# tansey/functionalmf

Measured on AMD Instinct MI355X. Metric: Gibbs sweeps/sec (full W+V update) at (512,256,64) K=5; % HBM roofline, higher is better.
Workload: dtype f64; 1 GPU; gaussian_btf c3 (512,256,64,4) nembeds=5 tf_order=2 complete data, W+V update, rng=device; burn_in_sweeps=10, step_loop=C side (btf_wv_steps: one call queues the K steps), v_sampler=spectral, likelihood_form=complete, parallelism=rows(W)/cols(V) x1

## Files before the change

### functionalmf_amd/csrc/btf_abi.hip

```cpp
#include "../../include/btf.h"
#include "btf_kernels.h"
#include "btf_banded_fast.h"
#include "btf_banded_twist.h"
#include "btf_banded_chunk.h"
#include "btf_spectral.h"
#include "btf_gass.h"
#include "btf_gass_ep.h"
#include "btf_gass_features.h"
#include "btf_gamma_grid.h"
#include "btf_fused.h"
#include "btf_functionals.h"
#include "btf_instances.h"
#include "btf_comm.h"
#include "btf_ctx.h"
#include <hip/hip_ext.h>
#include <unistd.h>

#include <algorithm>
#include <atomic>
#include <climits>
#include <cmath>
#include <cstdio>
#include <cstdlib>
#include <cstring>
// ... 142 lines not shown
  return BTF_OK;
}

inline int unr3_min_rpb() {
  static const int v = [] { const char* e = std::getenv("BTF_UNR3_RPB"); return e ? std::atoi(e) : 2048; }();
  return v;
}
inline bool lean_on() {
  static const bool v = [] { const char* e = std::getenv("BTF_ACC_LEAN"); return !e || std::atoi(e) != 0; }();
  return v;
}
template <int K>
void launch_accum(btf_ctx* c, int kid, int mode, const double* X, const double* Cx, const unsigned char* C8, const double* U,
                  const int* srcmap, int Rdim, int ld, int rpb, int nch, EigSide side = EigSide{nullptr, 0, 0, nullptr},
                  EigSideCols sidec = EigSideCols{nullptr, 0, CurveLists{nullptr, nullptr, nullptr}, nullptr, 0.0, nullptr},
                  TauSide tau = TauSide{}, GramSide gram = GramSide{},
                  ChunkMap cm = ChunkMap{0, 0, INT_MAX, 0, 0, 0}, SweepSide sw = SweepSide{},
                  const FuseW* fw = nullptr, const FuseV* fv = nullptr) {
  if (cm.row_end == 0) cm.row_end = Rdim;
  {
    static const double min_mb = [] { const char* e = std::getenv("BTF_NT_MIN_MB"); return e ? std::atof(e) : 100.0; }();
    cm.nt = (double)Rdim * (double)ld * 8.0 >= min_mb * 1048576.0 ? 1 : 0;
  }
#ifdef BTF_ACC_STAMPS
  cm.stamps = c->acc_stamps;
#endif
  Prof p(c, kid);
  const int cpw = TAU_SIDE_CPW;
  cm.nside = (sw.sc.hyp ? 1 : 0) + (sw.lam.hyp ? 1 : 0) + (side.out ? 1 + eig_side_groups(sidec.ncols, acc_waves(K, mode)) : 0) +
             (tau.Tau2 ? (tau.M + cpw - 1) / cpw : 0) + (gram.gpart ? gram.nblocks : 0) + (gram.sum_src ? 1 : 0) + (fw ? fw->owners : 0);
  dim3 grid((ld / ACC_TILE) * nch + cm.nside);
  if (fw || fv) {
    const bool unr3 = rpb >= unr3_min_rpb();
    if constexpr (K == 8) {
      if (unr3 && fw) { p.launch(accum_kernel<K, 0, 16, double, double, 3, 2, FUSE_W>, grid, dim3(16 * WAVE), 0, X, Cx, U, srcmap, c->part, Rdim, ld, rpb, side, sidec, tau, gram, cm, sw, *fw); return; }
      if (unr3 && fv) { p.launch(accum_kernel<K, 0, 16, double, double, 3, 2, FUSE_V>, grid, dim3(16 * WAVE), 0, X, Cx, U, srcmap, c->part, Rdim, ld, rpb, side, sidec, tau, gram, cm, sw, *fv); return; }
    }
    if constexpr (K <= 8) {
      if (fw) p.launch(accum_kernel<K, 0, 16, double, double, 0, 2, FUSE_W>, grid, dim3(16 * WAVE), 0, X, Cx, U, srcmap, c->part, Rdim, ld, rpb, side, sidec, tau, gram, cm, sw, *fw);
      else {
        const bool df_on = c->fused_dataflow != 0;
        FuseV f2 = *fv;
        constexpr int RG = K < 4 ? 4 : (K > 6 ? 6 : K);
        f2.dataflow = (df_on && f2.a.pband && f2.pimg && !f2.cnt && !f2.hp.flag && K <= 6 &&
                       vf_df_fits(f2.a.T, K, f2.a.TF, f2.a.nD, 16, RG)) ? 1 : 0;

        if constexpr (K <= 6) {
          if (f2.dataflow) { p.launch(accum_kernel<K, 0, 16, double, double, 0, 2, FUSE_VDF>, grid, dim3(16 * WAVE), 0, X, Cx, U, srcmap, c->part, Rdim, ld, rpb, side, sidec, tau, gram, cm, sw, f2); return; }
        }
        p.launch(accum_kernel<K, 0, 16, double, double, 0, 2, FUSE_V>, grid, dim3(16 * WAVE), 0, X, Cx, U, srcmap, c->part, Rdim, ld, rpb, side, sidec, tau, gram, cm, sw, f2);
      }
    }
    return;
  }
  const signed char* A8 = (mode >= 1 && !C8 && X == c->A_wT) ? c->A8_wT : ((mode >= 1 && !C8 && X == c->A_v) ? c->A8_v : nullptr);
  if (A8) {
    if (mode == 2) p.launch(accum_kernel<K, 2, acc_waves(K, 2), double, signed char>, grid, dim3(acc_waves(K, 2) * WAVE), 0, A8, Cx, U, srcmap, c->part, Rdim, ld, rpb, side, sidec, tau, gram, cm, sw, FuseNone{});
    else p.launch(accum_kernel<K, 1, acc_waves(K, 1), double, signed char>, grid, dim3(acc_waves(K, 1) * WAVE), 0, A8, Cx, U, srcmap, c->part, Rdim, ld, rpb, side, sidec, tau, gram, cm, sw, FuseNone{});
    return;
  }
  if (mode >= 1 && C8) {
    if (mode == 2) p.launch(accum_kernel<K, 2, acc_waves(K, 2), unsigned char>, grid, dim3(acc_waves(K, 2) * WAVE), 0, X, C8, U, srcmap, c->part, Rdim, ld, rpb, side, sidec, tau, gram, cm, sw, FuseNone{});
    else p.launch(accum_kernel<K, 1, acc_waves(K, 1), unsigned char>, grid, dim3(acc_waves(K, 1) * WAVE), 0, X, C8, U, srcmap, c->part, Rdim, ld, rpb, side, sidec, tau, gram, cm, sw, FuseNone{});
  } else if (mode == 2) p.launch(accum_kernel<K, 2>, grid, dim3(acc_waves(K, 2) * WAVE), 0, X, Cx, U, srcmap, c->part, Rdim, ld, rpb, side, sidec, tau, gram, cm, sw, FuseNone{});
  else if (mode == 1) p.launch(accum_kernel<K, 1>, grid, dim3(acc_waves(K, 1) * WAVE), 0, X, Cx, U, srcmap, c->part, Rdim, ld, rpb, side, sidec, tau, gram, cm, sw, FuseNone{});
  else if (K <= 8 && acc_waves(K, 0) == 16 && rpb < unr3_min_rpb() && !tau.Tau2 && !sw.sc.hyp && !sw.lam.hyp && lean_on()) {
    if constexpr (K <= 8) p.launch(accum_kernel<K, 0, 16, double, double, 0, 2, FUSE_LEAN>, grid, dim3(16 * WAVE), 0, X, Cx, U, srcmap, c->part, Rdim, ld, rpb, side, sidec, tau, gram, cm, sw, FuseNone{});
  }
  else if (K >= 10 && ACC_WAVES != acc_waves(10, 0) && !side.out && rpb < unr3_min_rpb()) {
    if constexpr (K >= 10) p.launch(accum_kernel<K, 0, ACC_WAVES>, grid, dim3(ACC_WAVES * WAVE), 0, X, Cx, U, srcmap, c->part, Rdim, ld, rpb, side, sidec, tau, gram, cm, sw, FuseNone{});
  }
  else if (rpb >= unr3_min_rpb()) p.launch(accum_kernel<K, 0, acc_waves(K, 0), double, double, 3>, grid, dim3(acc_waves(K, 0) * WAVE), 0, X, Cx, U, srcmap, c->part, Rdim, ld, rpb, side, sidec, tau, gram, cm, sw, FuseNone{});
  else p.launch(accum_kernel<K, 0>, grid, dim3(acc_waves(K, 0) * WAVE), 0, X, Cx, U, srcmap, c->part, Rdim, ld, rpb, side, sidec, tau, gram, cm, sw, FuseNone{});
}
struct PgPasses { bool flat, series, frac; int mode; };
PgPasses pg_passes(const btf_ctx* c) {
  PgPasses p{false, false, false, c->pg_mode};
  if (c->counts && p.mode == PG_MODE_DEFAULT) p.mode = PG_MODE_SERIES_ALL;
  if (p.mode == PG_MODE_SERIES_ALL) { p.series = true; return p; }
  if (p.mode == PG_MODE_EXACT_ALL) { p.flat = c->pg_has_small || c->pg_has_big; p.frac = c->pg_has_frac; }
  else { p.flat = c->pg_has_small; p.series = c->pg_has_big || c->pg_has_frac; }
  if (!p.flat && !p.series && !p.frac) p.series = true;
  return p;
}
template <int K>
void launch_pg(btf_ctx* c, const double* B, double* out, const double* Lf, const double* Uf, int nl, int ld, int Rdim,
               unsigned long long base, unsigned long long stride_r, unsigned long long stride_l, unsigned long long seed) {
  const int gx = (nl + PG_THREADS - 1) / PG_THREADS;
  int nrb = std::max(1, std::min(Rdim, 4096 / std::max(1, gx)));
  const int rpb = (Rdim + nrb - 1) / nrb;
  nrb = (Rdim + rpb - 1) / rpb;
  const PgPasses ps = pg_passes(c);
  int fill = 1;
  if (ps.flat) {
    Prof p(c, BTF_K_PG);
    const int rpx = round_up(rpb, PGX_CPL);
// ... 3766 lines not shown
```

### functionalmf_amd/csrc/btf_fused.h

```cpp
#pragma once
#include "btf_kernels.h"
#include "btf_spectral.h"

namespace btf {

__device__ __forceinline__ bool poll_flag(const unsigned* flag, unsigned epoch) {
  for (unsigned spins = 0; spins < (1u << 22); ++spins) {
    if (__hip_atomic_load((const gu32_t*)flag, __ATOMIC_RELAXED, __HIP_MEMORY_SCOPE_AGENT) == epoch) return true;
    __builtin_amdgcn_s_sleep(8);
  }
  return false;
}

struct HypPub { const double* pub; const unsigned* flag; unsigned epoch; int which; };

struct FuseW {
  WSolveArgs a;
  unsigned* cnt;
  unsigned expected;
  int owners;
  int rows;
  int rw;
  HypPub hp;
  const unsigned* gram_cnt; unsigned gram_expected;
// ... 771 lines not shown
template <> __device__ __forceinline__ unsigned* fuse_tickets<FUSE_VDF>(const FuseV& fz) { return nullptr; }
template <> __device__ __forceinline__ int fuse_chunks<FUSE_VDF>(const FuseV& fz) { return 1; }
template <> __device__ __forceinline__ int fuse_owners<FUSE_VDF>(const FuseV&) { return 0; }

__device__ __forceinline__ void df_signal(unsigned* c) {
  __builtin_amdgcn_fence(__ATOMIC_RELEASE, "workgroup");
  if ((threadIdx.x & 63) == 0) __hip_atomic_fetch_add(c, 1u, __ATOMIC_RELAXED, __HIP_MEMORY_SCOPE_WORKGROUP);
}
#ifndef BTF_DF_SLEEP
#define BTF_DF_SLEEP 1
#endif
template <int SLEEP = BTF_DF_SLEEP>
__device__ __forceinline__ void df_wait(unsigned* c, unsigned target, unsigned* bad) {
  bool seen = false;
  for (unsigned spins = 0; spins < (1u << 22) / SLEEP; ++spins) {
    if (__hip_atomic_load(c, __ATOMIC_RELAXED, __HIP_MEMORY_SCOPE_WORKGROUP) >= target) { seen = true; break; }
    __builtin_amdgcn_s_sleep(SLEEP);
  }
  if (!seen && (threadIdx.x & 63) == 0) __hip_atomic_store(bad, 1u, __ATOMIC_RELAXED, __HIP_MEMORY_SCOPE_WORKGROUP);
  __builtin_amdgcn_fence(__ATOMIC_ACQUIRE, "workgroup");
}

template <int K, int S>
__device__ __forceinline__ void v_df_begin(const FuseV& fv, int tile, double* lds, VDfPre& pre) {
  unsigned* cw = reinterpret_cast<unsigned*>(lds + vf_red_doubles(false) - VF_MAILBOX + 96);
  if (threadIdx.x < 64) cw[threadIdx.x] = 0u;
  __syncthreads();
  v_df_band_load<K, S>(fv, tile, pre);
}
template <int K, int S>
__device__ __forceinline__ void v_df_band_load(const FuseV& fv, int tile, VDfPre& pre) {
  const VSpecArgs& a = fv.a;
  const int T = a.T, NG = ACC_TILE / T;
  const int lane = threadIdx.x & 63;
  const int pw = __builtin_amdgcn_readfirstlane(threadIdx.x >> 6);
  const int cg = pw - NG, j = tile * NG + cg;
#pragma unroll
  for (int u = 0; u < 8; ++u) pre.pv[u] = make_double2(0.0, 0.0);
  if (pw >= NG && pw < 2 * NG && j < a.ml) {
    const int PB = df_layout(T, K, S).PB;
    const double2* src = reinterpret_cast<const double2*>(fv.pimg + (size_t)j * 2 * PB);
#pragma unroll
    for (int u = 0; u < 8; ++u)
      if (lane + 64 * u < PB) pre.pv[u] = src[lane + 64 * u];
  }
}
template <int K, int S>
__device__ __forceinline__ void v_df_band_store(const FuseV& fv, int tile, double* lds, const VDfPre& pre) {
  const VSpecArgs& a = fv.a;
  const int T = a.T, NG = ACC_TILE / T;
  const int lane = threadIdx.x & 63;
  const int pw = __builtin_amdgcn_readfirstlane(threadIdx.x >> 6);
  const int cg = pw - NG;
  if (!(pw >= NG && pw < 2 * NG && tile * NG + cg < a.ml)) return;
  const DfLayout D = df_layout(T, K, S);
  double2* dst = reinterpret_cast<double2*>(lds + vf_red_doubles(false) - VF_MAILBOX - (size_t)(cg + 1) * D.size + D.P);
#pragma unroll
  for (int u = 0; u < 8; ++u)
    if (lane + 64 * u < D.PB) dst[lane + 64 * u] = pre.pv[u];
  unsigned* cw = reinterpret_cast<unsigned*>(lds + vf_red_doubles(false) - VF_MAILBOX + 96);
  df_signal(cw + DFC_GROUP0 + cg * DFC_PER_GROUP + DFG_BAND);
}

template <int K, int S, int WAVES, int RG, int NVV>
__device__ __forceinline__ void v_fused_df(const FuseV& fv, int tile, double* lds, const double (&acc)[NVV][2], long long* stamps,
                                           const DfEarly& early) {
  static_assert(NVV == K && K <= RG, "one reduction round");
  static_assert(S == 3 && WAVES == 16, "tf_order 2, 16 waves");
  VSpecArgs a = fv.a;
  const int T = a.T, n = T * K, KK = tri(K);
  constexpr int D1 = S + 1, WN = S * (S + 1) + S;
  constexpr int NT = VF_GROUP_WAVES * WAVE;
  const int NG = ACC_TILE / T;
  const int Tp = T + S + 1;
  int nl, nr, ns;
  spectral_split(T, S, nl, nr, ns);
  const int lane = threadIdx.x & 63;
// ... 360 lines not shown
```

### functionalmf_amd/csrc/btf_instances.h

```cpp
#pragma once
#include "btf_kernels.h"
#include "btf_banded_twist.h"
#include "btf_spectral.h"
#include "btf_fused.h"

namespace btf {

#define BTF_ACC_ARGS_F(XT, CT, FZ) \
  (const XT*, const CT*, const double*, const int*, double*, int, int, int, EigSide, EigSideCols, TauSide, GramSide, ChunkMap, SweepSide, FZ)
#define BTF_ACC_ARGS(XT, CT) BTF_ACC_ARGS_F(XT, CT, FuseNone)
#define BTF_ACCUM_SET(P, K)                                                                              \
  P void accum_kernel<K, 0> BTF_ACC_ARGS(double, double);                                                \
  P void accum_kernel<K, 0, acc_waves(K, 0), double, double, 3> BTF_ACC_ARGS(double, double);            \
  P void accum_kernel<K, 1> BTF_ACC_ARGS(double, double);                                                \
  P void accum_kernel<K, 2> BTF_ACC_ARGS(double, double);                                                \
  P void accum_kernel<K, 1, acc_waves(K, 1), unsigned char> BTF_ACC_ARGS(double, unsigned char);         \
  P void accum_kernel<K, 2, acc_waves(K, 2), unsigned char> BTF_ACC_ARGS(double, unsigned char);         \
  P void accum_kernel<K, 1, acc_waves(K, 1), double, signed char> BTF_ACC_ARGS(signed char, double);     \
  P void accum_kernel<K, 2, acc_waves(K, 2), double, signed char> BTF_ACC_ARGS(signed char, double);

#define BTF_ACCUM_K10W_SET(P)                                                                            \
  P void accum_kernel<10, 0, ACC_WAVES> BTF_ACC_ARGS(double, double);

#define BTF_FUSED_W_SET(P, K)                                                                            \
  P void accum_kernel<K, 0, 16, double, double, 0, 2, FUSE_W> BTF_ACC_ARGS_F(double, double, FuseW);
#define BTF_FUSED_V_SET(P, K)                                                                            \
  P void accum_kernel<K, 0, 16, double, double, 0, 2, FUSE_V> BTF_ACC_ARGS_F(double, double, FuseV);
#define BTF_FUSED_VDF_SET(P, K)                                                                          \
  P void accum_kernel<K, 0, 16, double, double, 0, 2, FUSE_VDF> BTF_ACC_ARGS_F(double, double, FuseV);
#define BTF_LEAN_SET(P, K)                                                                               \
  P void accum_kernel<K, 0, 16, double, double, 0, 2, FUSE_LEAN> BTF_ACC_ARGS(double, double);
#define BTF_FUSED_UNR3_SET(P, K)                                                                         \
// ... 91 lines not shown
```

### functionalmf_amd/csrc/btf_kernels.h

```cpp
#pragma once
#include <type_traits>
#include "btf_device.h"
#include "btf_eig.h"
#include "btf_pg_exact.h"

namespace btf {

#ifndef BTF_ACC_WAVES
#define BTF_ACC_WAVES 16
#endif
#ifndef BTF_DF_UNR
#define BTF_DF_UNR 4
#endif
#ifndef BTF_DF_PREFETCH
#define BTF_DF_PREFETCH 1
#endif
#ifndef BTF_DF_SHARE
#define BTF_DF_SHARE 0
#endif
#ifndef BTF_ACC_UNR
#define BTF_ACC_UNR 2
#endif
#ifndef BTF_ACC_PF_WT
#define BTF_ACC_PF_WT 0
#endif
#ifndef BTF_ACC_UNR_WT
#define BTF_ACC_UNR_WT 2
#endif
#ifndef BTF_ACC_WAVES_WT
#define BTF_ACC_WAVES_WT 12
#endif
#ifndef BTF_ACC_WAVES_K10
#define BTF_ACC_WAVES_K10 8
#endif
#ifndef BTF_ACC_UNR_K9
#define BTF_ACC_UNR_K9 2
#endif
#ifndef BTF_ACC_ULDS_MINK
// ... 141 lines not shown

struct EigSideCols { const int* cols; int ncols; CurveLists cv; const double* W; double inv_R; double* eig_cols; };
__host__ __device__ constexpr int eig_side_tpw(int waves) { return waves >= 4 ? 4 : waves; }
__host__ __device__ constexpr int eig_side_groups(int ncols, int waves) { return (ncols + eig_side_tpw(waves) - 1) / eig_side_tpw(waves); }

struct TauSide {
  const double* V; int T, nD, M;
  const int* dr_ptr; const int* dr_col; const double* dr_val;
  double lam2, lo, hi;
  double* Tau2; double* Ta; double* Tb; double* Tc; double* lsum;
  unsigned long long seed; const double* hyp;
};
__device__ void tau2_column(const TauSide& t, int K, int j, int tid256, double* red4);
constexpr int TAU_SIDE_CPW = 2;

struct GramSide {
  const double* U; int Rdim; double* gpart; int nblocks; unsigned* cnt;
  const double* sum_src; int sum_n; double* sum_out; int sum_threads;
};

struct ChunkMap {
  int slot_base, row_base, skip_at, skip_rows, row_end; int nside;
  int nt;
#ifdef BTF_ACC_STAMPS
  long long* stamps;
#endif
};

struct ScalarSide {
  const double* sse_cols; int M; double sconst, nobs;
  const double* W; int NK; double nfree;
  double nu2_a, nu2_b, sig_a, sig_b; int which; unsigned long long seed; double* hyp;
  double* pub; unsigned* flag; unsigned epoch;
};
struct LamSide { const double* lsum; int M; double shape; int exact; unsigned long long seed; double* hyp; double* pub; unsigned* flag; unsigned epoch; };
struct SweepSide { ScalarSide sc; LamSide lam; };
struct BandSide {
  const double* Tau2; int nD;
  const int* st_ptr; const int* st_row; const double* st_coef;
  int TD1, col0, ml;
  double* pband; double* pimg; int img_T, img_D1, img_PB;
  const double* hyp; double lam2;
  const double* lam_pub; const unsigned* lam_flag; unsigned epoch;
  int* status;
};
__device__ inline void band_side(const BandSide& bs, int j, double* itau, int nthreads);
// ... 35 lines not shown
struct VPre;
template <int K, int S, int WAVES, int NSUM>
__device__ __forceinline__ void v_fused_tail(const FuseV& fv, int tile, double* lds, const double (&sums)[NSUM], int nv_round, int tv, int tc, long long* stamps,
                                             const VPre& pre, const double* mailbox, bool band_early, bool unr3);
template <int K, int S> __device__ __forceinline__ void v_fused_prefetch(const FuseV& fv, int tile, double* mailbox, VPre& pre, bool band_early);
template <int K, int S, class PRE> __device__ __forceinline__ void v_fused_prefetch_loads(const FuseV& fv, int tile, PRE& pre, bool band_early);
constexpr int VF_PRE = 4;
template <int K, int S> __device__ __forceinline__ bool v_fused_band_early(const FuseV& fv, int tile, double* lds, bool unr3);
#ifndef BTF_VF_BANDPRE
#define BTF_VF_BANDPRE 1
#endif
#if BTF_VF_BANDPRE
template <int K, int S> __device__ __forceinline__ bool v_fused_band_preload(const FuseV& fv, int tile, VPre& pre);
template <int K, int S> __device__ __forceinline__ void v_fused_band_store(const FuseV& fv, int tile, double* lds, const VPre& pre, bool unr3);
#endif
template <int FUSE> struct FusePre { struct type {}; };
constexpr int VF_MAILBOX_DOUBLES = 128;
struct VDfPre { double2 pv[8]; };
template <int FUSE> __device__ __forceinline__ int fuse_chain_waves(const typename FuseSel<FUSE>::type& fz) { return 0; }
struct DfEarly { double epub; bool have; };
template <int FUSE> __device__ __forceinline__ const unsigned* fuse_eig_flag(const typename FuseSel<FUSE>::type& fz) { return nullptr; }
template <int FUSE> __device__ __forceinline__ const double* fuse_eig_pub(const typename FuseSel<FUSE>::type& fz) { return nullptr; }
template <int FUSE> __device__ __forceinline__ unsigned fuse_epoch(const typename FuseSel<FUSE>::type& fz) { return 0u; }
template <int K, int S> __device__ __forceinline__ void v_df_begin(const FuseV& fv, int tile, double* lds, VDfPre& pre);
template <int K, int S> __device__ __forceinline__ void v_df_band_load(const FuseV& fv, int tile, VDfPre& pre);
template <int K, int S> __device__ __forceinline__ void v_df_band_store(const FuseV& fv, int tile, double* lds, const VDfPre& pre);
template <int K, int S, int WAVES, int RG, int NVV>
__device__ __forceinline__ void v_fused_df(const FuseV& fv, int tile, double* lds, const double (&acc)[NVV][2], long long* stamps, const DfEarly& early);
template <int FUSE> __device__ __forceinline__ unsigned* fuse_tickets(const typename FuseSel<FUSE>::type& fz);
template <int FUSE> __device__ __forceinline__ int fuse_chunks(const typename FuseSel<FUSE>::type& fz);
__device__ __forceinline__ bool last_arriver_of(unsigned* cnt, unsigned expected, unsigned* word) {
  if (threadIdx.x == 0) {
    const unsigned t = __hip_atomic_fetch_add((gu32_t*)cnt, 1u, __ATOMIC_RELAXED, __HIP_MEMORY_SCOPE_AGENT);
    const bool last = t + 1u == expected;
    if (last) __hip_atomic_store((gu32_t*)cnt, 0u, __ATOMIC_RELAXED, __HIP_MEMORY_SCOPE_AGENT);
    *word = last ? 1u : 0u;
  }
  __syncthreads();
  const bool last = *word != 0u;
  __syncthreads();
  return last;
}
__host__ __device__ constexpr int vf_red_doubles(bool unr3) { return unr3 ? 15360 : 18432; }
__host__ __device__ constexpr int w_tail_lds_doubles(int K);
__host__ __device__ constexpr int w_owner_lds_budget(int K);

#ifdef BTF_ACC_STAMPS
#define ACC_STAMP(i) do { if (threadIdx.x == 0 && b < 4096 && cm.stamps) cm.stamps[b * 8 + (i)] = wall_clock64(); } while (0)
#define ACC_SIDE_STAMP(i) do { if (threadIdx.x == 0 && cm.stamps) cm.stamps[(4096 + blockIdx.x) * 8 + (i)] = wall_clock64(); } while (0)
#define ACC_TAIL_STAMPS (cm.stamps && b < 4096 ? cm.stamps + b * 8 : nullptr)
#define ACC_OWNER_STAMPS (cm.stamps ? cm.stamps + (size_t)(4096 + blockIdx.x) * 8 : nullptr)
#else
#define ACC_STAMP(i) do { } while (0)
#define ACC_SIDE_STAMP(i) do { } while (0)
#define ACC_TAIL_STAMPS nullptr
#define ACC_OWNER_STAMPS nullptr
#endif
#define TAIL_STAMP(st, i) do { if ((st) && threadIdx.x == 0) (st)[i] = wall_clock64(); } while (0)
template <int K, int MODE, int WAVES = acc_waves(K, MODE), typename CT = double, typename XT = double, int UNRV = 0,
          int OPL = acc_opl(K, MODE), int FUSE = FUSE_NONE>
__global__ __launch_bounds__(WAVES * WAVE) BTF_ACC_EU_ATTR(K, MODE, WAVES, FUSE) void accum_kernel(
    const XT* __restrict__ X, const CT* __restrict__ Cx, const double* __restrict__ U,
    const int* __restrict__ srcmap, double* __restrict__ part, int Rdim, int ld,
    int rows_per_block, EigSide side, EigSideCols sidec, TauSide tau, GramSide gram, ChunkMap cm, SweepSide sw,
    typename FuseSel<FUSE>::type fz) {
  static_assert(FUSE == FUSE_NONE || (MODE == 0 && OPL == 2 && WAVES == 16), "the fused tails follow the complete-data stream");
  constexpr bool PLAIN = FUSE == FUSE_NONE || FUSE == FUSE_LEAN;
  constexpr int KK = tri(K);
  constexpr int NV = MODE == 0 ? K : K + KK;
  constexpr int ACC_WAVES = WAVES;
  constexpr int ACC_UNR = FUSE == FUSE_VDF ? BTF_DF_UNR : (UNRV > 0 ? UNRV : (MODE >= 1 ? BTF_ACC_UNR_WT : (K >= 9 ? BTF_ACC_UNR_K9 : BTF_ACC_UNR)));
  constexpr int ACC_RGT = WAVES * WAVE / ACC_TILE, ACC_RGL = (96 * 1024) / (WAVES * ACC_TILE * 8);
  constexpr int ACC_RG0 = ACC_RGT < 4 ? ACC_RGT : 4;
  constexpr int ACC_RGW = ACC_RGT < ACC_RGL ? (ACC_RGT < NV ? ACC_RGT : NV) : (ACC_RGL < NV ? ACC_RGL : NV);
  constexpr int ACC_RG = ACC_RGW > ACC_RG0 ? ACC_RGW : ACC_RG0;
  constexpr int RED_SLOT = ACC_RG * ACC_TILE;
  constexpr int RED_SLOTS = (FUSE == FUSE_V || FUSE == FUSE_VDF) ? (vf_red_doubles(UNRV == 3) + RED_SLOT - 1) / RED_SLOT : ACC_WAVES;
  static_assert(RED_SLOTS >= ACC_WAVES, "reduction scratch");
  __shared__ double red[RED_SLOTS][ACC_RG][ACC_TILE];
  static_assert(FUSE != FUSE_W || (w_tail_lds_doubles(K) <= WAVES * ACC_RG * ACC_TILE && w_owner_lds_budget(K) == WAVES * ACC_RG * ACC_TILE), "W owner scratch");
  constexpr bool ULDS = MODE == 0 && K >= BTF_ACC_ULDS_MINK && UNRV == 3;
  constexpr int ACC_UROWS_MAX = 512;
  __shared__ double ush[ULDS ? ACC_UROWS_MAX * K : 1];

  const int lane = threadIdx.x & 63;
  const int wave = __builtin_amdgcn_readfirstlane(threadIdx.x >> 6);
  int b = blockIdx.x;
  if (b < cm.nside) {
  if constexpr (FUSE == FUSE_W) {
    const int nown = fuse_owners<FUSE>(fz);
    if (b < nown) {
      ACC_SIDE_STAMP(0);
      w_fused_owner<K, WAVES>(fz, b, &red[0][0][0], ACC_OWNER_STAMPS);
      ACC_SIDE_STAMP(3);
      return;
    }
    b -= nown;
  }
  if constexpr (FUSE != FUSE_LEAN) {
  if (sw.sc.hyp) {
    if (b == 0) { sweep_scalar_side<WAVES>(sw.sc, &red[0][0][0]); return; }
    b -= 1;
  }
  if (sw.lam.hyp) {
    if (b == 0) { sweep_lam_side<WAVES>(sw.lam, &red[0][0][0]); return; }
    b -= 1;
  }
  }
  if (side.out) {
    constexpr int TPW = eig_side_tpw(WAVES);
    const int nside = 1 + eig_side_groups(sidec.ncols, WAVES);
// ... 76 lines not shown
      if ((int)threadIdx.x < gram.sum_threads && l < lanes) {
        double sg = 0.0;
        for (int b0 = l; b0 < gram.sum_n; b0 += 8 * lanes) {
          double x[8];
#pragma unroll
          for (int u = 0; u < 8; ++u) x[u] = b0 + u * lanes < gram.sum_n ? gram.sum_src[(size_t)(b0 + u * lanes) * KK + q] : 0.0;
#pragma unroll
          for (int u = 0; u < 8; ++u) sg += x[u];
        }
        scratch[l * KK + q] = sg;
      }
      __syncthreads();
      if ((int)threadIdx.x < KK) {
        double t = 0.0;
        for (int bb = 0; bb < lanes; ++bb) t += scratch[bb * KK + threadIdx.x];
        gram.sum_out[threadIdx.x] = t;
      }
      return;
    }
    b -= 1;
  }
  return;
  }
  b -= cm.nside;
  ACC_STAMP(0);
  const int ntiles = ld / ACC_TILE;
  const int lchunk = b / ntiles, tile = b - lchunk * ntiles;
  const int chunk = cm.slot_base + lchunk;
  static_assert(OPL == 2 || (OPL == 1 && WAVES % 2 == 0), "outputs per lane");
  constexpr int NWR = OPL == 2 ? WAVES : WAVES / 2;
  const int half = OPL == 2 ? 0 : (wave & 1);
  const int wv = OPL == 2 ? wave : (wave >> 1);
  const size_t col = (size_t)tile * ACC_TILE + (OPL == 2 ? 2 * lane : 64 * half + lane);
  int r0 = cm.row_base + lchunk * rows_per_block;
  if (r0 >= cm.skip_at) r0 += cm.skip_rows;
  const int r1 = min(r0 + rows_per_block, cm.row_end);

  constexpr bool dataflow = FUSE == FUSE_VDF;
  static_assert(!dataflow || (UNRV != 3 && NV <= ACC_RG && OPL == 2), "the dataflow tail: one reduction round, two rows in flight");
  bool df_band_done = false;
  DfEarly df_early{0.0, false};
  VDfPre dfpre;
  if constexpr (dataflow) v_df_begin<K, 3>(fz, tile, &red[0][0][0], dfpre);
  int df_ncw = 0;
  if constexpr (dataflow) df_ncw = fuse_chain_waves<FUSE>(fz);
  int nwr_rt = NWR;
  bool band_early = false;
  if constexpr (FUSE == FUSE_V) band_early = v_fused_band_early<K, 3>(fz, tile, &red[0][0][0], UNRV == 3);
  typename FusePre<FUSE>::type vpre;
#if BTF_VF_BANDPRE
  if constexpr (FUSE == FUSE_V) band_early = v_fused_band_preload<K, 3>(fz, tile, vpre);
#endif
  double acc[NV][OPL];
#pragma unroll
  for (int v = 0; v < NV; ++v)
#pragma unroll
    for (int o = 0; o < OPL; ++o) acc[v][o] = 0.0;
#ifdef BTF_NO_NT
  constexpr bool nt = false;
#else
  const bool nt = __builtin_amdgcn_readfirstlane(cm.nt) != 0;
#endif
  int s0 = 0, s1 = 0;
  bool gram_on = true, gram_any = true;
  if constexpr (MODE == 2) {
    s0 = srcmap[col];
    if constexpr (OPL == 2) s1 = srcmap[col + 1];
    const bool own = s0 == (int)col || (OPL == 2 && s1 == (int)col + 1);
    gram_on = __builtin_amdgcn_readfirstlane(__any(own) ? 1 : 0) != 0;
    if constexpr (OPL == 1) gram_any = __syncthreads_or(own ? 1 : 0) != 0;
    else gram_any = gram_on;
  }
  int cs_form = 0, cs_src = 0;
  if constexpr (MODE == 2 && OPL == 2) {
    cs_src = __builtin_amdgcn_readfirstlane(s0);
    if (__all(s0 == cs_src && s1 == cs_src)) cs_form = 1;
    else if (__all(s1 == s0 + 1 && (s0 & 1) == 0)) cs_form = 2;
    cs_form = __builtin_amdgcn_readfirstlane(cs_form);
  }

  int ublk0 = r0;
  struct Rows { double2 x[ACC_UNR]; double2 c[MODE >= 1 ? ACC_UNR : 1]; double2 cs[MODE == 2 ? ACC_UNR : 1]; double uk[ACC_UNR][K]; };
  auto load_rows = [&](int rb, Rows& R, auto full, auto ntc) {
    constexpr bool FULL = decltype(full)::value;
// ... 121 lines not shown
      if (!nextB) break;
      more = rb + STEP < full_end;
      if (more) load_rows(rb + STEP, A, std::true_type{}, ntc);
      compute(rb, B);
      rb += STEP;
    }
  } else {
    if constexpr (FUSE == FUSE_V) {
      const int pre_end = full_end - VF_PRE * STEP;
      for (; rb < pre_end; rb += STEP) {
        Rows A;
        load_rows(rb, A, std::true_type{}, ntc);
        compute(rb, A);
      }
      v_fused_prefetch_loads<K, 3>(fz, tile, vpre, band_early);
    }
    if constexpr (dataflow) {
      const int g1 = NWR * ACC_UNR;
      const int rsplit = r0 + ((r1 - r0) * BTF_DF_SHARE / 100) / g1 * g1;
      nwr_rt = NWR;
      for (rb = r0 + wv; rb < rsplit; rb += g1) {
        Rows A;
        load_rows(rb, A, std::true_type{}, ntc);
        compute(rb, A);
        if (!df_band_done) { v_df_band_store<K, 3>(fz, tile, &red[0][0][0], dfpre); df_band_done = true; }
      }
      if (wave >= df_ncw) {
        nwr_rt = NWR - df_ncw;
        const int step = nwr_rt * ACC_UNR, fend = r1 - (ACC_UNR - 1) * nwr_rt;
        const bool eigw = BTF_DF_PREFETCH && wave == df_ncw;
        const int rprobe = r0 + (r1 - r0) * 5 / 8;
        unsigned eflag = 0u;
        int estate = 0;
        for (rb = rsplit + wv - df_ncw; rb < fend; rb += step) {
          Rows A;
          load_rows(rb, A, std::true_type{}, ntc);
          if (eigw && estate < 2 && rb >= rprobe) {
            if (estate == 1 && eflag == fuse_epoch<FUSE>(fz)) {
              if (lane < K + K * K) df_early.epub = load_sc1(fuse_eig_pub<FUSE>(fz) + lane);
              df_early.have = true;
              estate = 2;
            } else {
              eflag = __hip_atomic_load(fuse_eig_flag<FUSE>(fz), __ATOMIC_RELAXED, __HIP_MEMORY_SCOPE_AGENT);
              estate = 1;
            }
          }
          compute(rb, A);
          if (!df_band_done) { v_df_band_store<K, 3>(fz, tile, &red[0][0][0], dfpre); df_band_done = true; }
        }
        if (rb < r1) {
          Rows A;
          load_rows(rb, A, std::false_type{}, ntc);
          compute(rb, A);
        }
      }
      rb = r1;
    }
    for (; rb < full_end; rb += STEP) {
      Rows A;
      load_rows(rb, A, std::true_type{}, ntc);
      compute(rb, A);
    }
  }
  if constexpr (!ULDS) {
    if (rb < r1) {
      Rows A;
      load_rows(rb, A, std::false_type{}, ntc);
      compute(rb, A);
    }
  }

  };
  if (nt) run_stream(std::true_type{}); else run_stream(std::false_type{});
  ACC_STAMP(2);
  if constexpr (dataflow) {
    if (!df_band_done) {
      v_df_band_load<K, 3>(fz, tile, dfpre);
      v_df_band_store<K, 3>(fz, tile, &red[0][0][0], dfpre);
    }
    v_fused_df<K, 3, WAVES, ACC_RG, NV>(fz, tile, &red[0][0][0], acc, ACC_TAIL_STAMPS, df_early);
    return;
  }
  if constexpr (FUSE == FUSE_V) {
    if constexpr (ULDS) v_fused_prefetch_loads<K, 3>(fz, tile, vpre, band_early);
#if BTF_VF_BANDPRE
    if (band_early) v_fused_band_store<K, 3>(fz, tile, &red[0][0][0], vpre, UNRV == 3);
#endif
    v_fused_prefetch<K, 3>(fz, tile, &red[0][0][0] + RED_SLOTS * RED_SLOT - VF_MAILBOX_DOUBLES, vpre, band_early);
  }
  const int tv = threadIdx.x >> 7;
  const int tc = threadIdx.x & 127;
  constexpr int NFS = PLAIN ? 1 : (NV + ACC_RG - 1) / ACC_RG;
  double fsum[NFS];
#pragma unroll
  for (int r = 0; r < NFS; ++r) fsum[r] = 0.0;
#pragma unroll
  for (int g = 0; g < NV; g += ACC_RG) {
    if (MODE == 2 && !gram_any && g >= K) break;
#pragma unroll
    for (int v = 0; v < ACC_RG; ++v) {
      if (g + v < NV) {
// ... 2341 lines not shown
```

Baseline: 26790 sweeps/s.

## Repack accum kernel arguments into a compact preloaded head and defer dataflow LDS init

Reorders and compresses the accumulate kernel's argument list so the hot scalars (pointers, ld, rows, row_end, packed nside/flags/T code) fit in a fixed 14-dword head. The intent is that the kernel reads them from preloaded SGPRs instead of loading ChunkMap and FuseV fields from the kernarg segment. Row remapping is now skipped behind a flag, and the dataflow band load takes pimg, T and ml directly. The mailbox-zeroing barrier in v_df_begin is moved until after the first row loads are issued, so it no longer stalls the stream start. The risks are the ABI change across every instance and a changed placement of __syncthreads relative to the loads.

Result: no change. 26980 sweeps/s, median of 2 (+0.7%).

```diff
diff --git a/functionalmf_amd/csrc/btf_abi.hip b/functionalmf_amd/csrc/btf_abi.hip
--- a/functionalmf_amd/csrc/btf_abi.hip
+++ b/functionalmf_amd/csrc/btf_abi.hip
@@ -188,22 +188,26 @@
     static const double min_mb = [] { const char* e = std::getenv("BTF_NT_MIN_MB"); return e ? std::atof(e) : 100.0; }();
     cm.nt = (double)Rdim * (double)ld * 8.0 >= min_mb * 1048576.0 ? 1 : 0;
   }
+  AccRest rest{cm.slot_base, cm.row_base, cm.skip_at, cm.skip_rows};
+  const bool remap = cm.slot_base != 0 || cm.row_base != 0 || cm.skip_rows != 0;
+  const unsigned long long aux2 = (unsigned long long)reinterpret_cast<uintptr_t>(srcmap);
 #ifdef BTF_ACC_STAMPS
-  cm.stamps = c->acc_stamps;
+  rest.stamps = c->acc_stamps;
 #endif
   Prof p(c, kid);
   const int cpw = TAU_SIDE_CPW;
   cm.nside = (sw.sc.hyp ? 1 : 0) + (sw.lam.hyp ? 1 : 0) + (side.out ? 1 + eig_side_groups(sidec.ncols, acc_waves(K, mode)) : 0) +
              (tau.Tau2 ? (tau.M + cpw - 1) / cpw : 0) + (gram.gpart ? gram.nblocks : 0) + (gram.sum_src ? 1 : 0) + (fw ? fw->owners : 0);
   dim3 grid((ld / ACC_TILE) * nch + cm.nside);
+  const unsigned nside_flags = ((unsigned)cm.nside << ACC_F_BITS) | (cm.nt ? ACC_F_NT : 0u) | (remap ? ACC_F_REMAP : 0u);
   if (fw || fv) {
     const bool unr3 = rpb >= unr3_min_rpb();
     if constexpr (K == 8) {
-      if (unr3 && fw) { p.launch(accum_kernel<K, 0, 16, double, double, 3, 2, FUSE_W>, grid, dim3(16 * WAVE), 0, X, Cx, U, srcmap, c->part, Rdim, ld, rpb, side, sidec, tau, gram, cm, sw, *fw); return; }
-      if (unr3 && fv) { p.launch(accum_kernel<K, 0, 16, double, double, 3, 2, FUSE_V>, grid, dim3(16 * WAVE), 0, X, Cx, U, srcmap, c->part, Rdim, ld, rpb, side, sidec, tau, gram, cm, sw, *fv); return; }
+      if (unr3 && fw) { p.launch(accum_kernel<K, 0, 16, double, double, 3, 2, FUSE_W>, grid, dim3(16 * WAVE), 0, X, U, c->part, (const void*)Cx, aux2, ld, rpb, cm.row_end, nside_flags, rest, side, sidec, tau, gram, sw, *fw); return; }
+      if (unr3 && fv) { p.launch(accum_kernel<K, 0, 16, double, double, 3, 2, FUSE_V>, grid, dim3(16 * WAVE), 0, X, U, c->part, (const void*)Cx, aux2, ld, rpb, cm.row_end, nside_flags, rest, side, sidec, tau, gram, sw, *fv); return; }
     }
     if constexpr (K <= 8) {
-      if (fw) p.launch(accum_kernel<K, 0, 16, double, double, 0, 2, FUSE_W>, grid, dim3(16 * WAVE), 0, X, Cx, U, srcmap, c->part, Rdim, ld, rpb, side, sidec, tau, gram, cm, sw, *fw);
+      if (fw) p.launch(accum_kernel<K, 0, 16, double, double, 0, 2, FUSE_W>, grid, dim3(16 * WAVE), 0, X, U, c->part, (const void*)Cx, aux2, ld, rpb, cm.row_end, nside_flags, rest, side, sidec, tau, gram, sw, *fw);
       else {
         const bool df_on = c->fused_dataflow != 0;
         FuseV f2 = *fv;
@@ -212,32 +216,33 @@
                        vf_df_fits(f2.a.T, K, f2.a.TF, f2.a.nD, 16, RG)) ? 1 : 0;
 
         if constexpr (K <= 6) {
-          if (f2.dataflow) { p.launch(accum_kernel<K, 0, 16, double, double, 0, 2, FUSE_VDF>, grid, dim3(16 * WAVE), 0, X, Cx, U, srcmap, c->part, Rdim, ld, rpb, side, sidec, tau, gram, cm, sw, f2); return; }
+          if (f2.dataflow) { p.launch(accum_kernel<K, 0, 16, double, double, 0, 2, FUSE_VDF>, grid, dim3(16 * WAVE), 0, X, U, c->part, (const void*)f2.pimg, (unsigned long long)f2.a.ml, ld, rpb, cm.row_end,
+                                      nside_flags | (acc_depth_code(f2.a.T) << ACC_F_T_SHIFT), rest, side, sidec, tau, gram, sw, f2); return; }
         }
-        p.launch(accum_kernel<K, 0, 16, double, double, 0, 2, FUSE_V>, grid, dim3(16 * WAVE), 0, X, Cx, U, srcmap, c->part, Rdim, ld, rpb, side, sidec, tau, gram, cm, sw, f2);
+        p.launch(accum_kernel<K, 0, 16, double, double, 0, 2, FUSE_V>, grid, dim3(16 * WAVE), 0, X, U, c->part, (const void*)Cx, aux2, ld, rpb, cm.row_end, nside_flags, rest, side, sidec, tau, gram, sw, f2);
       }
     }
     return;
   }
   const signed char* A8 = (mode >= 1 && !C8 && X == c->A_wT) ? c->A8_wT : ((mode >= 1 && !C8 && X == c->A_v) ? c->A8_v : nullptr);
   if (A8) {
-    if (mode == 2) p.launch(accum_kernel<K, 2, acc_waves(K, 2), double, signed char>, grid, dim3(acc_waves(K, 2) * WAVE), 0, A8, Cx, U, srcmap, c->part, Rdim, ld, rpb, side, sidec, tau, gram, cm, sw, FuseNone{});
-    else p.launch(accum_kernel<K, 1, acc_waves(K, 1), double, signed char>, grid, dim3(acc_waves(K, 1) * WAVE), 0, A8, Cx, U, srcmap, c->part, Rdim, ld, rpb, side, sidec, tau, gram, cm, sw, FuseNone{});
+    if (mode == 2) p.launch(accum_kernel<K, 2, acc_waves(K, 2), double, signed char>, grid, dim3(acc_waves(K, 2) * WAVE), 0, A8, U, c->part, (const void*)Cx, aux2, ld, rpb, cm.row_end, nside_flags, rest, side, sidec, tau, gram, sw, FuseNone{});
+    else p.launch(accum_kernel<K, 1, acc_waves(K, 1), double, signed char>, grid, dim3(acc_waves(K, 1) * WAVE), 0, A8, U, c->part, (const void*)Cx, aux2, ld, rpb, cm.row_end, nside_flags, rest, side, sidec, tau, gram, sw, FuseNone{});
     return;
   }
   if (mode >= 1 && C8) {
-    if (mode == 2) p.launch(accum_kernel<K, 2, acc_waves(K, 2), unsigned char>, grid, dim3(acc_waves(K, 2) * WAVE), 0, X, C8, U, srcmap, c->part, Rdim, ld, rpb, side, sidec, tau, gram, cm, sw, FuseNone{});
-    else p.launch(accum_kernel<K, 1, acc_waves(K, 1), unsigned char>, grid, dim3(acc_waves(K, 1) * WAVE), 0, X, C8, U, srcmap, c->part, Rdim, ld, rpb, side, sidec, tau, gram, cm, sw, FuseNone{});
-  } else if (mode == 2) p.launch(accum_kernel<K, 2>, grid, dim3(acc_waves(K, 2) * WAVE), 0, X, Cx, U, srcmap, c->part, Rdim, ld, rpb, side, sidec, tau, gram, cm, sw, FuseNone{});
-  else if (mode == 1) p.launch(accum_kernel<K, 1>, grid, dim3(acc_waves(K, 1) * WAVE), 0, X, Cx, U, srcmap, c->part, Rdim, ld, rpb, side, sidec, tau, gram, cm, sw, FuseNone{});
+    if (mode == 2) p.launch(accum_kernel<K, 2, acc_waves(K, 2), unsigned char>, grid, dim3(acc_waves(K, 2) * WAVE), 0, X, U, c->part, (const void*)C8, aux2, ld, rpb, cm.row_end, nside_flags, rest, side, sidec, tau, gram, sw, FuseNone{});
+    else p.launch(accum_kernel<K, 1, acc_waves(K, 1), unsigned char>, grid, dim3(acc_waves(K, 1) * WAVE), 0, X, U, c->part, (const void*)C8, aux2, ld, rpb, cm.row_end, nside_flags, rest, side, sidec, tau, gram, sw, FuseNone{});
+  } else if (mode == 2) p.launch(accum_kernel<K, 2>, grid, dim3(acc_waves(K, 2) * WAVE), 0, X, U, c->part, (const void*)Cx, aux2, ld, rpb, cm.row_end, nside_flags, rest, side, sidec, tau, gram, sw, FuseNone{});
+  else if (mode == 1) p.launch(accum_kernel<K, 1>, grid, dim3(acc_waves(K, 1) * WAVE), 0, X, U, c->part, (const void*)Cx, aux2, ld, rpb, cm.row_end, nside_flags, rest, side, sidec, tau, gram, sw, FuseNone{});
   else if (K <= 8 && acc_waves(K, 0) == 16 && rpb < unr3_min_rpb() && !tau.Tau2 && !sw.sc.hyp && !sw.lam.hyp && lean_on()) {
-    if constexpr (K <= 8) p.launch(accum_kernel<K, 0, 16, double, double, 0, 2, FUSE_LEAN>, grid, dim3(16 * WAVE), 0, X, Cx, U, srcmap, c->part, Rdim, ld, rpb, side, sidec, tau, gram, cm, sw, FuseNone{});
+    if constexpr (K <= 8) p.launch(accum_kernel<K, 0, 16, double, double, 0, 2, FUSE_LEAN>, grid, dim3(16 * WAVE), 0, X, U, c->part, (const void*)Cx, aux2, ld, rpb, cm.row_end, nside_flags, rest, side, sidec, tau, gram, sw, FuseNone{});
   }
   else if (K >= 10 && ACC_WAVES != acc_waves(10, 0) && !side.out && rpb < unr3_min_rpb()) {
-    if constexpr (K >= 10) p.launch(accum_kernel<K, 0, ACC_WAVES>, grid, dim3(ACC_WAVES * WAVE), 0, X, Cx, U, srcmap, c->part, Rdim, ld, rpb, side, sidec, tau, gram, cm, sw, FuseNone{});
-  }
-  else if (rpb >= unr3_min_rpb()) p.launch(accum_kernel<K, 0, acc_waves(K, 0), double, double, 3>, grid, dim3(acc_waves(K, 0) * WAVE), 0, X, Cx, U, srcmap, c->part, Rdim, ld, rpb, side, sidec, tau, gram, cm, sw, FuseNone{});
-  else p.launch(accum_kernel<K, 0>, grid, dim3(acc_waves(K, 0) * WAVE), 0, X, Cx, U, srcmap, c->part, Rdim, ld, rpb, side, sidec, tau, gram, cm, sw, FuseNone{});
+    if constexpr (K >= 10) p.launch(accum_kernel<K, 0, ACC_WAVES>, grid, dim3(ACC_WAVES * WAVE), 0, X, U, c->part, (const void*)Cx, aux2, ld, rpb, cm.row_end, nside_flags, rest, side, sidec, tau, gram, sw, FuseNone{});
+  }
+  else if (rpb >= unr3_min_rpb()) p.launch(accum_kernel<K, 0, acc_waves(K, 0), double, double, 3>, grid, dim3(acc_waves(K, 0) * WAVE), 0, X, U, c->part, (const void*)Cx, aux2, ld, rpb, cm.row_end, nside_flags, rest, side, sidec, tau, gram, sw, FuseNone{});
+  else p.launch(accum_kernel<K, 0>, grid, dim3(acc_waves(K, 0) * WAVE), 0, X, U, c->part, (const void*)Cx, aux2, ld, rpb, cm.row_end, nside_flags, rest, side, sidec, tau, gram, sw, FuseNone{});
 }
 struct PgPasses { bool flat, series, frac; int mode; };
 PgPasses pg_passes(const btf_ctx* c) {
diff --git a/functionalmf_amd/csrc/btf_fused.h b/functionalmf_amd/csrc/btf_fused.h
--- a/functionalmf_amd/csrc/btf_fused.h
+++ b/functionalmf_amd/csrc/btf_fused.h
@@ -817,37 +817,34 @@
 }
 
 template <int K, int S>
-__device__ __forceinline__ void v_df_begin(const FuseV& fv, int tile, double* lds, VDfPre& pre) {
+__device__ __forceinline__ void v_df_begin(double* lds) {
   unsigned* cw = reinterpret_cast<unsigned*>(lds + vf_red_doubles(false) - VF_MAILBOX + 96);
   if (threadIdx.x < 64) cw[threadIdx.x] = 0u;
   __syncthreads();
-  v_df_band_load<K, S>(fv, tile, pre);
 }
 template <int K, int S>
-__device__ __forceinline__ void v_df_band_load(const FuseV& fv, int tile, VDfPre& pre) {
-  const VSpecArgs& a = fv.a;
-  const int T = a.T, NG = ACC_TILE / T;
+__device__ __forceinline__ void v_df_band_load(const double* pimg, int T, int ml, int tile, VDfPre& pre) {
+  const int NG = df_cols_per_tile(T);
   const int lane = threadIdx.x & 63;
   const int pw = __builtin_amdgcn_readfirstlane(threadIdx.x >> 6);
   const int cg = pw - NG, j = tile * NG + cg;
 #pragma unroll
   for (int u = 0; u < 8; ++u) pre.pv[u] = make_double2(0.0, 0.0);
-  if (pw >= NG && pw < 2 * NG && j < a.ml) {
+  if (pw >= NG && pw < 2 * NG && j < ml) {
     const int PB = df_layout(T, K, S).PB;
-    const double2* src = reinterpret_cast<const double2*>(fv.pimg + (size_t)j * 2 * PB);
+    const double2* src = reinterpret_cast<const double2*>(pimg + (size_t)j * 2 * PB);
 #pragma unroll
     for (int u = 0; u < 8; ++u)
       if (lane + 64 * u < PB) pre.pv[u] = src[lane + 64 * u];
   }
 }
 template <int K, int S>
-__device__ __forceinline__ void v_df_band_store(const FuseV& fv, int tile, double* lds, const VDfPre& pre) {
-  const VSpecArgs& a = fv.a;
-  const int T = a.T, NG = ACC_TILE / T;
+__device__ __forceinline__ void v_df_band_store(int T, int ml, int tile, double* lds, const VDfPre& pre) {
+  const int NG = df_cols_per_tile(T);
   const int lane = threadIdx.x & 63;
   const int pw = __builtin_amdgcn_readfirstlane(threadIdx.x >> 6);
   const int cg = pw - NG;
-  if (!(pw >= NG && pw < 2 * NG && tile * NG + cg < a.ml)) return;
+  if (!(pw >= NG && pw < 2 * NG && tile * NG + cg < ml)) return;
   const DfLayout D = df_layout(T, K, S);
   double2* dst = reinterpret_cast<double2*>(lds + vf_red_doubles(false) - VF_MAILBOX - (size_t)(cg + 1) * D.size + D.P);
 #pragma unroll
diff --git a/functionalmf_amd/csrc/btf_instances.h b/functionalmf_amd/csrc/btf_instances.h
--- a/functionalmf_amd/csrc/btf_instances.h
+++ b/functionalmf_amd/csrc/btf_instances.h
@@ -6,8 +6,8 @@
 
 namespace btf {
 
-#define BTF_ACC_ARGS_F(XT, CT, FZ) \
-  (const XT*, const CT*, const double*, const int*, double*, int, int, int, EigSide, EigSideCols, TauSide, GramSide, ChunkMap, SweepSide, FZ)
+#define BTF_ACC_ARGS_F(XT, CT, FZ)  \
+  (const XT*, const double*, double*, const void*, unsigned long long, int, int, int, unsigned, AccRest, EigSide, EigSideCols, TauSide, GramSide, SweepSide, FZ)
 #define BTF_ACC_ARGS(XT, CT) BTF_ACC_ARGS_F(XT, CT, FuseNone)
 #define BTF_ACCUM_SET(P, K)                                                                              \
   P void accum_kernel<K, 0> BTF_ACC_ARGS(double, double);                                                \
diff --git a/functionalmf_amd/csrc/btf_kernels.h b/functionalmf_amd/csrc/btf_kernels.h
--- a/functionalmf_amd/csrc/btf_kernels.h
+++ b/functionalmf_amd/csrc/btf_kernels.h
@@ -14,6 +14,9 @@
 #endif
 #ifndef BTF_DF_PREFETCH
 #define BTF_DF_PREFETCH 1
+#endif
+#ifndef BTF_DF_BEGIN_EARLY
+#define BTF_DF_BEGIN_EARLY 0
 #endif
 #ifndef BTF_DF_SHARE
 #define BTF_DF_SHARE 0
@@ -201,6 +204,15 @@
 struct ChunkMap {
   int slot_base, row_base, skip_at, skip_rows, row_end; int nside;
   int nt;
+#ifdef BTF_ACC_STAMPS
+  long long* stamps;
+#endif
+};
+enum : unsigned { ACC_F_NT = 1u, ACC_F_REMAP = 2u, ACC_F_T_SHIFT = 2u, ACC_F_T_MASK = 3u, ACC_F_BITS = 4u };
+__host__ __device__ constexpr unsigned acc_depth_code(int T) { return T == 32 ? 1u : (T == 64 ? 2u : (T == 128 ? 3u : 0u)); }
+constexpr int ACC_HEAD_DWORDS = 14;
+struct AccRest {
+  int slot_base, row_base, skip_at, skip_rows;
 #ifdef BTF_ACC_STAMPS
   long long* stamps;
 #endif
@@ -282,9 +294,10 @@
 template <int FUSE> __device__ __forceinline__ const unsigned* fuse_eig_flag(const typename FuseSel<FUSE>::type& fz) { return nullptr; }
 template <int FUSE> __device__ __forceinline__ const double* fuse_eig_pub(const typename FuseSel<FUSE>::type& fz) { return nullptr; }
 template <int FUSE> __device__ __forceinline__ unsigned fuse_epoch(const typename FuseSel<FUSE>::type& fz) { return 0u; }
-template <int K, int S> __device__ __forceinline__ void v_df_begin(const FuseV& fv, int tile, double* lds, VDfPre& pre);
-template <int K, int S> __device__ __forceinline__ void v_df_band_load(const FuseV& fv, int tile, VDfPre& pre);
-template <int K, int S> __device__ __forceinline__ void v_df_band_store(const FuseV& fv, int tile, double* lds, const VDfPre& pre);
+template <int K, int S> __device__ __forceinline__ void v_df_begin(double* lds);
+template <int K, int S> __device__ __forceinline__ void v_df_band_load(const double* pimg, int T, int ml, int tile, VDfPre& pre);
+template <int K, int S> __device__ __forceinline__ void v_df_band_store(int T, int ml, int tile, double* lds, const VDfPre& pre);
+__device__ __forceinline__ int df_cols_per_tile(int T) { return ACC_TILE >> __builtin_ctz((unsigned)(T | ACC_TILE)); }
 template <int K, int S, int WAVES, int RG, int NVV>
 __device__ __forceinline__ void v_fused_df(const FuseV& fv, int tile, double* lds, const double (&acc)[NVV][2], long long* stamps, const DfEarly& early);
 template <int FUSE> __device__ __forceinline__ unsigned* fuse_tickets(const typename FuseSel<FUSE>::type& fz);
@@ -306,10 +319,10 @@
 __host__ __device__ constexpr int w_owner_lds_budget(int K);
 
 #ifdef BTF_ACC_STAMPS
-#define ACC_STAMP(i) do { if (threadIdx.x == 0 && b < 4096 && cm.stamps) cm.stamps[b * 8 + (i)] = wall_clock64(); } while (0)
-#define ACC_SIDE_STAMP(i) do { if (threadIdx.x == 0 && cm.stamps) cm.stamps[(4096 + blockIdx.x) * 8 + (i)] = wall_clock64(); } while (0)
-#define ACC_TAIL_STAMPS (cm.stamps && b < 4096 ? cm.stamps + b * 8 : nullptr)
-#define ACC_OWNER_STAMPS (cm.stamps ? cm.stamps + (size_t)(4096 + blockIdx.x) * 8 : nullptr)
+#define ACC_STAMP(i) do { if (threadIdx.x == 0 && b < 4096 && rest.stamps) rest.stamps[b * 8 + (i)] = wall_clock64(); } while (0)
+#define ACC_SIDE_STAMP(i) do { if (threadIdx.x == 0 && rest.stamps) rest.stamps[(4096 + blockIdx.x) * 8 + (i)] = wall_clock64(); } while (0)
+#define ACC_TAIL_STAMPS (rest.stamps && b < 4096 ? rest.stamps + b * 8 : nullptr)
+#define ACC_OWNER_STAMPS (rest.stamps ? rest.stamps + (size_t)(4096 + blockIdx.x) * 8 : nullptr)
 #else
 #define ACC_STAMP(i) do { } while (0)
 #define ACC_SIDE_STAMP(i) do { } while (0)
@@ -320,10 +333,17 @@
 template <int K, int MODE, int WAVES = acc_waves(K, MODE), typename CT = double, typename XT = double, int UNRV = 0,
           int OPL = acc_opl(K, MODE), int FUSE = FUSE_NONE>
 __global__ __launch_bounds__(WAVES * WAVE) BTF_ACC_EU_ATTR(K, MODE, WAVES, FUSE) void accum_kernel(
-    const XT* __restrict__ X, const CT* __restrict__ Cx, const double* __restrict__ U,
-    const int* __restrict__ srcmap, double* __restrict__ part, int Rdim, int ld,
-    int rows_per_block, EigSide side, EigSideCols sidec, TauSide tau, GramSide gram, ChunkMap cm, SweepSide sw,
+    const XT* __restrict__ X, const double* __restrict__ U, double* __restrict__ part, const void* __restrict__ aux,
+    unsigned long long aux2, int ld, int rows_per_block, int row_end, unsigned nside_flags,
+    AccRest rest, EigSide side, EigSideCols sidec, TauSide tau, GramSide gram, SweepSide sw,
     typename FuseSel<FUSE>::type fz) {
+  static_assert(sizeof(X) + sizeof(U) + sizeof(part) + sizeof(aux) + sizeof(aux2) + sizeof(ld) + sizeof(rows_per_block) +
+                sizeof(row_end) + sizeof(nside_flags) == 4 * ACC_HEAD_DWORDS, "the head is the preloaded window");
+  const CT* __restrict__ Cx = static_cast<const CT*>(aux);
+  const int* __restrict__ srcmap = reinterpret_cast<const int*>(aux2);
+  const int ncols = (int)aux2;
+  const int nside = (int)(nside_flags >> ACC_F_BITS);
+  const unsigned flags = nside_flags;
   static_assert(FUSE == FUSE_NONE || (MODE == 0 && OPL == 2 && WAVES == 16), "the fused tails follow the complete-data stream");
   constexpr bool PLAIN = FUSE == FUSE_NONE || FUSE == FUSE_LEAN;
   constexpr int KK = tri(K);
@@ -346,7 +366,7 @@
   const int lane = threadIdx.x & 63;
   const int wave = __builtin_amdgcn_readfirstlane(threadIdx.x >> 6);
   int b = blockIdx.x;
-  if (b < cm.nside) {
+  if (b < nside) {
   if constexpr (FUSE == FUSE_W) {
     const int nown = fuse_owners<FUSE>(fz);
     if (b < nown) {
@@ -469,28 +489,41 @@
   }
   return;
   }
-  b -= cm.nside;
+  b -= nside;
   ACC_STAMP(0);
   const int ntiles = ld / ACC_TILE;
   const int lchunk = b / ntiles, tile = b - lchunk * ntiles;
-  const int chunk = cm.slot_base + lchunk;
   static_assert(OPL == 2 || (OPL == 1 && WAVES % 2 == 0), "outputs per lane");
   constexpr int NWR = OPL == 2 ? WAVES : WAVES / 2;
   const int half = OPL == 2 ? 0 : (wave & 1);
   const int wv = OPL == 2 ? wave : (wave >> 1);
   const size_t col = (size_t)tile * ACC_TILE + (OPL == 2 ? 2 * lane : 64 * half + lane);
-  int r0 = cm.row_base + lchunk * rows_per_block;
-  if (r0 >= cm.skip_at) r0 += cm.skip_rows;
-  const int r1 = min(r0 + rows_per_block, cm.row_end);
+  int r0 = lchunk * rows_per_block, chunk = lchunk;
+  if (flags & ACC_F_REMAP) {
+    asm volatile("" ::: "memory");
+    r0 += rest.row_base;
+    if (r0 >= rest.skip_at) r0 += rest.skip_rows;
+    chunk += rest.slot_base;
+  }
+  const int r1 = min(r0 + rows_per_block, row_end);
 
   constexpr bool dataflow = FUSE == FUSE_VDF;
   static_assert(!dataflow || (UNRV != 3 && NV <= ACC_RG && OPL == 2), "the dataflow tail: one reduction round, two rows in flight");
   bool df_band_done = false;
   DfEarly df_early{0.0, false};
   VDfPre dfpre;
-  if constexpr (dataflow) v_df_begin<K, 3>(fz, tile, &red[0][0][0], dfpre);
+  const double* df_pimg = static_cast<const double*>(aux);
+  const int df_T = 16 << ((flags >> ACC_F_T_SHIFT) & ACC_F_T_MASK);
+  bool df_begun = false;
+  auto df_begin_once = [&]() {
+    if constexpr (dataflow) {
+      if (!df_begun) { v_df_begin<K, 3>(&red[0][0][0]); df_begun = true; }
+    }
+  };
+  if constexpr (dataflow) v_df_band_load<K, 3>(df_pimg, df_T, ncols, tile, dfpre);
+  if (BTF_DF_BEGIN_EARLY) df_begin_once();
   int df_ncw = 0;
-  if constexpr (dataflow) df_ncw = fuse_chain_waves<FUSE>(fz);
+  if constexpr (dataflow) df_ncw = df_cols_per_tile(df_T);
   int nwr_rt = NWR;
   bool band_early = false;
   if constexpr (FUSE == FUSE_V) band_early = v_fused_band_early<K, 3>(fz, tile, &red[0][0][0], UNRV == 3);
@@ -506,7 +539,7 @@
 #ifdef BTF_NO_NT
   constexpr bool nt = false;
 #else
-  const bool nt = __builtin_amdgcn_readfirstlane(cm.nt) != 0;
+  const bool nt = (flags & ACC_F_NT) != 0;
 #endif
   int s0 = 0, s1 = 0;
   bool gram_on = true, gram_any = true;
@@ -674,8 +707,9 @@
       for (rb = r0 + wv; rb < rsplit; rb += g1) {
         Rows A;
         load_rows(rb, A, std::true_type{}, ntc);
+        df_begin_once();
         compute(rb, A);
-        if (!df_band_done) { v_df_band_store<K, 3>(fz, tile, &red[0][0][0], dfpre); df_band_done = true; }
+        if (!df_band_done) { v_df_band_store<K, 3>(df_T, ncols, tile, &red[0][0][0], dfpre); df_band_done = true; }
       }
       if (wave >= df_ncw) {
         nwr_rt = NWR - df_ncw;
@@ -687,6 +721,7 @@
         for (rb = rsplit + wv - df_ncw; rb < fend; rb += step) {
           Rows A;
           load_rows(rb, A, std::true_type{}, ntc);
+          df_begin_once();
           if (eigw && estate < 2 && rb >= rprobe) {
             if (estate == 1 && eflag == fuse_epoch<FUSE>(fz)) {
               if (lane < K + K * K) df_early.epub = load_sc1(fuse_eig_pub<FUSE>(fz) + lane);
@@ -698,7 +733,7 @@
             }
           }
           compute(rb, A);
-          if (!df_band_done) { v_df_band_store<K, 3>(fz, tile, &red[0][0][0], dfpre); df_band_done = true; }
+          if (!df_band_done) { v_df_band_store<K, 3>(df_T, ncols, tile, &red[0][0][0], dfpre); df_band_done = true; }
         }
         if (rb < r1) {
           Rows A;
@@ -706,6 +741,7 @@
           compute(rb, A);
         }
       }
+      df_begin_once();
       rb = r1;
     }
     for (; rb < full_end; rb += STEP) {
@@ -727,8 +763,8 @@
   ACC_STAMP(2);
   if constexpr (dataflow) {
     if (!df_band_done) {
-      v_df_band_load<K, 3>(fz, tile, dfpre);
-      v_df_band_store<K, 3>(fz, tile, &red[0][0][0], dfpre);
+      v_df_band_load<K, 3>(df_pimg, df_T, ncols, tile, dfpre);
+      v_df_band_store<K, 3>(df_T, ncols, tile, &red[0][0][0], dfpre);
     }
     v_fused_df<K, 3, WAVES, ACC_RG, NV>(fz, tile, &red[0][0][0], acc, ACC_TAIL_STAMPS, df_early);
     return;
```
